# YuyaW-0118/Sparse-Matrix-Linear-Equations

Measured on AMD Instinct MI355X. Metric: fp64 SpMV GFLOP/s + achieved HBM GB/s vs roofline; CG iters/sec, higher is better.
Workload: dtype f64; 1 GPU; merge-path CSR SpMV fp64, 1 RHS, batch of 4 pwtk-shaped matrices per step per GPU (configs[1]); m=217918, nnz=11524432, batch=4, parallelism=independent SpMV batches, 1 GPU(s)

## Files before the change

sparse-matrix-linear-equations_amd/csrc/mspmv_internal.h:

```cpp
#pragma once

#include <hip/hip_runtime.h>

#include <cstdint>
#include <map>
#include <string>
#include <type_traits>
#include <utility>
#include <vector>

#include "mspmv.h"
#include "mspmv_host.h"

static inline hipError_t memset_sync(void *p, int value, size_t bytes)
{
    const hipError_t e = hipMemset(p, value, bytes);
    return e == hipSuccess ? hipStreamSynchronize(nullptr) : e;
}

namespace mspmv {

constexpr int kBlock = 256;
constexpr unsigned kFaultTicket = 1u;
constexpr int kNnzPad = 16;
// ... 214 lines not shown
    double last_tile_kernel_ms = 0.0;
    int last_kernels_per_call = 1;
    void *d_flush = nullptr;
    size_t flush_cap = 0;
    mspmv::ResidentCg *rcg = nullptr;
    std::string last_cg_kernel;
    std::string last_solver_product;
    int spmv_onewave = -1;
    int spmv_slab = -1;
    int spmv_runs = -1;
    int spmm_slab[5] = {-1, -1, -1, -1, -1};
    int dia = -1;
};

namespace mspmv {
mspmv_status host_pattern(mspmv_handle_s *h, const int **ro, const int **ci);
bool host_pattern_resident(const mspmv_handle_s *h);
struct PatternScope {
    mspmv_handle_s *h;
    bool own;
    explicit PatternScope(mspmv_handle_s *hh) : h(hh), own(!hh->pat_scope) { hh->pat_scope = true; }
    ~PatternScope()
    {
        if (own) {
            h->pat_scope = false;
            std::vector<int>().swap(h->pat_ro);
            std::vector<int>().swap(h->pat_ci);
        }
    }
};
}

namespace mspmv {

struct TriFactor {
    unsigned long long gen = mspmv_next_generation();
    int device = 0;
    int n = 0;
    int *d_lro = nullptr, *d_lci = nullptr;
    double *d_lva = nullptr;
    int *d_uro = nullptr, *d_uci = nullptr;
    double *d_uva = nullptr;
    int *d_fwd_order = nullptr;
    int *d_bwd_order = nullptr;
    double *d_y = nullptr;
    size_t y_cap = 0;
    int num_colors = 0;
    bool l_diag = false;
    std::vector<int> color_off, perm;
    std::vector<int> lmax, umax;
    int *d_perm = nullptr;
};

}

struct mspmv_ic0_s : mspmv::TriFactor {};
struct mspmv_ilu0_s : mspmv::TriFactor {
    double *d_hat = nullptr;
    size_t hat_cap = 0;
};

namespace mspmv {

hipError_t tri_apply(const TriFactor *t, const double *d_src, double *d_dst, int L, CgControl *ctrl, hipStream_t s);
hipError_t tri_solve(const TriFactor *t, int which, const double *d_b, double *d_x, int L, CgControl *ctrl,
                     hipStream_t s);
mspmv_status tri_workspace(TriFactor *t, size_t elems, const char *what);
mspmv_status ilu0_workspace(mspmv_ilu0_s *ilu, size_t elems);
void tri_graph_key(const TriFactor *t, std::vector<const void *> &key);
hipError_t launch_color_trsv(const TriFactor *t, bool upper, const double *d_b, double *d_x, int L,
                             const CgControl *ctrl, hipStream_t s);
hipError_t launch_color_apply(const TriFactor *t, const double *d_src, double *d_dst, int L, const CgControl *ctrl,
                              hipStream_t s);

constexpr int kSlabPlanKey = -1;
constexpr int kRunPlanKey = -2;
mspmv_status build_slab_plan(mspmv_handle_s *h, TilePlan &p, double min_nnz_per_block = 0.0, int cfg = 0,
                             bool groups = false, int num_groups = 0);
void free_slab(SlabData *s);
hipError_t launch_slab(mspmv_handle_s *h, const TilePlan &plan, const double *d_x, double *d_y);
std::string slab_kernel_name(const mspmv_handle_s *h);
inline int slab_mm_key(int L) { return -(1 << 20) - L; }
const SlabMmCfg &slab_mm_cfg(int L, int which = -1);
mspmv_status build_slab_mm_plan(mspmv_handle_s *h, int L, TilePlan &p);
hipError_t launch_slab_mm(mspmv_handle_s *h, const TilePlan &plan, const double *d_X, double *d_Y, int L, int ld,
                          const CgControl *ctrl);
std::string slab_mm_kernel_name(const mspmv_handle_s *h, const TilePlan &plan);
mspmv_status plan_split_rows(TilePlan &p, const std::vector<int2> &hb, const std::vector<unsigned char> &hs);

constexpr int kDiaPlanKey = -3;
mspmv_status build_dia_plan(mspmv_handle_s *h, TilePlan &p, double min_fill, double min_window_fill);
void free_dia(DiaData *d);
hipError_t launch_dia(mspmv_handle_s *h, const TilePlan &plan, const double *d_X, double *d_Y, int L, int ld,
                      const CgControl *ctrl, double *partials = nullptr, long long row_off = 0,
                      hipStream_t stream = nullptr);
std::string dia_kernel_name(const mspmv_handle_s *h, int L);
hipError_t launch_cg1_dia(mspmv_handle_s *h, const TilePlan &plan, const double *rp_old, double *rp_new, double *d_x,
                          int parity, int nblk, double tol, int *nslots);
hipError_t launch_cg1_tile(mspmv_handle_s *h, const TilePlan &plan, const double *rp_old, double *rp_new, double *d_x,
                           int parity, int nblk, double tol, int *nslots);
bool dia_spmm_enabled();
bool dia_dot_fused();

hipError_t launch_merge_coords(const int *d_row_offsets, int m, int nnz, long long diag_step, int num_parts,
                               int2 *d_out, hipStream_t s);
hipError_t launch_tile_modes(const int *d_row_offsets, const int2 *d_bounds, const unsigned char *d_split,
                             int num_tiles, int L, unsigned char *d_modes, hipStream_t s, int lanes = kBlock);
int spmv_items_per_thread();
inline int l_index(int L) { return L == 1 ? 0 : L == 2 ? 1 : L == 4 ? 2 : L == 8 ? 3 : 4; }
hipError_t launch_snap(const int *d_row_offsets, int m, int2 *d_bounds, unsigned char *d_split, int num_tiles,
                       int snap, hipStream_t s);
hipError_t launch_pack_cols16(const int *d_cols, const int2 *d_bounds, int num_tiles, int *d_colbase,
                              unsigned short *d_cols16, hipStream_t s);
bool spmv_blocks_enabled();
bool spmm_blk_enabled();
constexpr int kBlkRunRows = 6;
constexpr int kBlkPerTile = 64;
constexpr int kBlkPlanChunks = 16;
constexpr int kBlkTileChunks = 8;
hipError_t launch_build_blocks(const int *d_row_offsets, const int *d_cols, const int2 *d_bounds,
                               const unsigned char *d_split, const int *d_colbase, int num_tiles, uint4 *d_blk,
                               hipStream_t s, int max_chunks = 8);
hipError_t launch_fill_pcols(const uint4 *d_blk, int blk_stride, const int2 *d_bounds,
                             const unsigned short *d_cols16, int num_tiles, unsigned short *d_pcols, hipStream_t s);
constexpr int kRecDwords = 16;
constexpr int kRecEntries = 12;
constexpr unsigned kRecEscape = 1u << 7;

__host__ __device__ inline int blk_rec_pos(int di)
{
    return (di & ~7) | ((di & 3) << 1) | ((di >> 2) & 1);
}

__host__ __device__ inline bool blk_rec_encode(const unsigned short *P, int wc, unsigned *ent)
{
    for (int e = 0; e < kRecEntries; ++e)
        ent[e] = 0u;
    int ne = 0;
    for (int q = 0; q < wc;) {
        int len = 1;
        while (q + len < wc && (int)P[q + len] == (int)P[q] + len)
            ++len;
        if (ne == kRecEntries) {
            for (int e = 0; e < kRecEntries; ++e)
                ent[e] = 0u;
            return false;
        }
        ent[ne++] = (unsigned)P[q] | ((unsigned)len << 16) | ((unsigned)q << 24);
        q += len;
    }
    return true;
}

template <typename F>
__host__ __device__ inline unsigned blk_rec_find(F &&ent, int q, int &e)
{
    e = 0;
    unsigned E = ent(0);
#pragma unroll
    for (int step = 8; step > 0; step >>= 1) {
        const int c = e + step;
        const bool in = c < kRecEntries;
        const unsigned Ec = ent(in ? c : e);
        if (in && (int)((Ec - 1u) >> 24) <= q) {
            e = c;
            E = Ec;
        }
    }
    return E;
}

__host__ __device__ inline unsigned blk_rec_decode(const unsigned *ent, int wc, int q)
{
    q = q < wc ? q : wc - 1;
    q = q < 0 ? 0 : q;
    int e;
    const unsigned E = blk_rec_find([&](int i) { return ent[i]; }, q, e);
    return (E & 0xffffu) + (unsigned)q - (E >> 24);
}

hipError_t launch_fill_recs(const uint4 *d_blk, int blk_stride, const unsigned short *d_pcols, int num_tiles,
                            unsigned *d_recs, int *d_counts, hipStream_t s);
hipError_t launch_build_dict(const int *d_cols, const int2 *d_bounds, int num_tiles, int max_items, int *d_dict,
                             int *d_ndict, unsigned short *d_idx16, hipStream_t s, bool multi, int L = 1);
constexpr int kSpmmDictBytes = 16384;
constexpr int kSpmmDict8Bytes = 0;
constexpr int spmm_dict_bytes(int L) { return L == 16 ? kSpmmDictBytes : L == 8 ? kSpmmDict8Bytes : 0; }
constexpr int spmm_dict_max(int L) { return spmm_dict_bytes(L) / (8 * L); }
hipError_t launch_spmm(mspmv_handle_s *h, const TilePlan &plan, const double *d_X, double *d_Y, int L,
                       int *kernels_launched, int ld = 0);
hipError_t launch_panel_copy(const double *src, int lds, double *dst, int ldd, long long rows, int cols, int dcols,
                             hipStream_t s);
hipError_t launch_spmm_tile_only(mspmv_handle_s *h, const TilePlan &plan, const double *d_X, double *d_Y, int L,
                                 int ld = 0, CgControl *ctrl = nullptr);
int tile_items_for(int L);
inline int plan_key(int L) { return L == 16 ? tile_items_for(16) + 1 : tile_items_for(L); }
int spmv_tile_blocks_per_cu();
hipError_t launch_stream_read(const double *p, size_t bytes, int num_cus, hipStream_t s);
std::string spmv_kernel_name(const mspmv_handle_s *h);
std::string spmm_kernel_name(const mspmv_handle_s *h, const TilePlan &plan, int L);
std::string solver_product_kernel_name(const mspmv_handle_s *h, const TilePlan &plan, const TilePlan *splan, int L);
bool stream_nt(const mspmv_handle_s *h);

using NativeWidths = std::integer_sequence<int, 1, 2, 4, 8, 16>;
template <typename F, int... N>
inline hipError_t dispatch_width(int L, F &&f, std::integer_sequence<int, N...>)
{
    hipError_t e = hipErrorInvalidValue;
    (void)((L == N && ((e = f(std::integral_constant<int, N>{})), true)) || ...);
    return e;
}
template <typename F>
inline hipError_t dispatch_L(int L, F &&f)
{
    return dispatch_width(L, f, NativeWidths{});
}
inline bool supported_L(int L)
{
    return dispatch_L(L, [](auto) { return hipSuccess; }) == hipSuccess;
}
template <typename F>
inline auto dispatch_bool(bool flag, F &&f)
{
    return flag ? f(std::true_type{}) : f(std::false_type{});
}

hipError_t launch_cg_init(mspmv_handle_s *h, const double *d_b, double *d_x, int L, double tol, int nblk);
hipError_t launch_spmv_tile_stamped(mspmv_handle_s *h, const TilePlan &plan, const double *d_x, double *d_y,
                                   unsigned long long *d_stamps);
hipError_t launch_cg_iteration(mspmv_handle_s *h, const TilePlan &plan, const TilePlan *splan, bool dot_fused,
                               double *d_x, int L, int parity, int nblk, double tol);
int cg_update_blocks(long long elems, int num_cus);
hipError_t launch_solver_product(mspmv_handle_s *h, const TilePlan &plan, const TilePlan *splan, const double *d_X,
                                 double *d_Y, int L);
hipError_t launch_bicgstab_init(mspmv_handle_s *h, const double *d_b, double *d_x, int L, double tol, int nblk);
hipError_t launch_bicgstab_iteration(mspmv_handle_s *h, const TilePlan &plan, const TilePlan *splan, double *d_x, int L,
                                     int nblk, double tol);
hipError_t launch_pbicgstab_iteration(mspmv_handle_s *h, mspmv_ilu0_s *ilu, const TilePlan &plan,
                                      const TilePlan *splan, double *d_x, int L, int nblk, double tol);
int cg_batch_iters(long long m, long long nnz, int L);
bool cg_split_iteration(int L);
int cg1_blocks(long long m);
hipError_t launch_cg1_init(mspmv_handle_s *h, const double *d_b, double *d_x, int nblk);
hipError_t launch_cg1_finish(mspmv_handle_s *h, double *d_x, int parity, int nblk);
bool cg_resident_enabled();
bool cg_resident_pipelined();
mspmv_status resident_prepare(mspmv_handle_s *h, ResidentCg **out);
void resident_free(ResidentCg *r);
hipError_t launch_cg_resident(mspmv_handle_s *h, ResidentCg *r, const double *d_b, double *d_x, int max_iters,
                              double tol, unsigned long long *d_stamps = nullptr, int stamp_iters = 0);
hipError_t launch_cg_xflush(mspmv_handle_s *h, double *d_x, int L, int nblk);
inline void consumer_level(int nslots, int stop, int L, long long *off, int *count)
{
    long long o = 0;
    int c = nslots;
    while (c > stop) {
        o += (long long)c * L;
        c = (c + kSlotGroup - 1) / kSlotGroup;
    }
    *off = o;
    *count = c;
}

struct CgVecArgs {
    long long n_elems;
    double *x;
    double *r;
    const double *p;
    double *p0;
    const double *ap;
    CgScalars *scal;
    CgControl *ctrl;
    unsigned char *conv;
    double *partials;
    double *hist;
    int hist_cap;
    double tol;
    const double *red_in;
    double *red_out;
    unsigned *gtickets;
    int pcg;
    int lazy_x;
    int rev;
};
enum class CgVecPass {
    InitPartials,
    InitFinish,
    PUpdate,
    XrUpdate,
    Finish,
};
hipError_t launch_dist_vec(CgVecPass pass, const CgVecArgs &a, int L, int nblk, double *p, hipStream_t s);
hipError_t launch_dist_pack(const double *p, const int *idx, long long n_elems, int L, double *send,
                            const CgControl *ctrl, hipStream_t s);
hipError_t launch_spmm_dot(mspmv_handle_s *h, const TilePlan &plan, const double *d_X, double *d_Y, int L,
                           CgControl *ctrl, double *partials, unsigned *gtickets, double *dot_out,
                           CgScalars *scal = nullptr, const unsigned char *conv = nullptr, int fold_mode = -1);
hipError_t launch_spmm_dot_tiles(mspmv_handle_s *h, const TilePlan &plan, const double *d_X, double *d_Y, int L,
                                 CgControl *ctrl, double *partials, hipStream_t s, long long row_off);
hipError_t launch_fold_dot(int T, int L, double *partials, unsigned *gtickets, double *dot_out, CgScalars *scal,
                           const unsigned char *conv, CgControl *ctrl, int fold_mode, hipStream_t s);
mspmv_status solver_plan(mspmv_handle_s *h, int L, const TilePlan **out);
mspmv_status product_plan(mspmv_handle_s *h, int L, const TilePlan **out);
mspmv_status window_plan(mspmv_handle_s *h, int L, const TilePlan **out);
void free_plan(TilePlan &p);
void drop_plans(mspmv_handle_s *h);
inline int native_chunk(int left)
{
    int w = 16;
    while (w > left)
        w >>= 1;
    return w;
}
mspmv_status csr_create_on_stream(const mspmv_csr_d *host, int device, hipStream_t stream, mspmv_handle *out);
mspmv_status csr_create_view(mspmv_handle parent, int row_lo, int row_hi, const int *host_row_offsets,
                             mspmv_handle *out);
mspmv_status time_spmm_batch(int count, const mspmv_handle *hs, const double *const *d_X, double *const *d_Y, int L,
                             int reps, double *step_ms, double *tile_kernel_ms, int *kernels_per_step, bool overlap);
hipError_t launch_pcg_init(mspmv_handle_s *h, mspmv_handle_s *hm, const TilePlan &mplan, const double *d_b,
                           double *d_x, int L, double tol, int nblk);
hipError_t launch_pcg_iteration(mspmv_handle_s *h, mspmv_handle_s *hm, const TilePlan &plan, const TilePlan &mplan,
                                double *d_x, int L, int nblk, double tol);
hipError_t launch_pcg_ic0_init(mspmv_handle_s *h, mspmv_ic0_s *ic, const double *d_b, double *d_x, int L, double tol,
                               int nblk);
hipError_t launch_pcg_ic0_iteration(mspmv_handle_s *h, mspmv_ic0_s *ic, const TilePlan &plan, double *d_x, int L,
                                    int nblk, double tol);
inline size_t partials_capacity(size_t slots, int L) { return (slots + slots / (kSlotGroup - 1) + 8) * L; }
inline size_t gtickets_capacity(size_t slots) { return (slots / (kSlotGroup - 1) + 8) * kTicketStride; }

#define HIP_TRY(expr)                                                                              \
// ... 63 lines not shown
```

sparse-matrix-linear-equations_amd/csrc/mspmv_kernels.hip:

```cpp
#include "mspmv_internal.h"
#include "mspmv_device.h"

#include <algorithm>
#include <type_traits>
#include <cmath>
#include <cstdio>
#include <cstdlib>

namespace mspmv {


template <typename... KArgs, typename... Args>
static void ggl(void (*kernel)(KArgs...), dim3 grid, dim3 block, hipStream_t s, Args... args)
{
    hipLaunchKernelGGL(kernel, grid, block, 0, s, args...);
}

template <bool NT, typename T>
__device__ __forceinline__ T ld_stream(const T *p)
{
    if (NT)
        return __builtin_nontemporal_load(p);
    return *p;
}
// ... 548 lines not shown
        const int q = q0 + (int)threadIdx.x + TB * (ubase + u);
        if (q > qlast)
            continue;
        const int k0 = W * q - n0;
#pragma unroll
        for (int e = 0; e < W; ++e) {
            const double v = (e & 1) ? st.v[u][e >> 1].y : st.v[u][e >> 1].x;
            if (k0 + e >= 0 && k0 + e < nnzt)
                s_prod[pslot(k0 + e)] = v * st.x[u][e];
        }
    }
}

template <int NJ, bool CG, bool NT>
__device__ __forceinline__ void stage_products(const TileArgs &a, int n0, int nnzt, double beta, double *s_prod)
{
    StageRegs<NJ, CG> st;
    stage_issue<NJ, CG, NT>(a, n0, nnzt, -1, st);
    stage_store<NJ, CG>(st, nnzt, beta, s_prod);
}

template <int NJ, bool NT, int TB>
__device__ __forceinline__ void dict_stage(const TileArgs &a, double *s_prod, int nd, int n0, int nnzt)
{
    constexpr int DJ = 3;
    const int tid = threadIdx.x;
    int ix[NJ];
    double v[NJ];
    int dc[DJ];
    double dx[DJ];
#pragma unroll
    for (int u = 0; u < DJ; ++u)
        dc[u] = ld_stream<NT>(a.dict + n0 + min(tid + u * TB, nd - 1));
#pragma unroll
    for (int j = 0; j < NJ; ++j)
        ix[j] = ld_stream<NT>(a.idx16 + n0 + min(tid + j * TB, nnzt - 1));
#pragma unroll
    for (int j = 0; j < NJ; ++j)
        v[j] = ld_stream<NT>(a.vals + n0 + min(tid + j * TB, nnzt - 1));
#pragma unroll
    for (int u = 0; u < DJ; ++u)
        dx[u] = a.x[dc[u]];
    double *s_x = s_prod;
#pragma unroll
    for (int u = 0; u < DJ; ++u)
        if (tid + u * TB < nd)
            s_x[tid + u * TB] = dx[u];
    for (int d = tid + DJ * TB; d < nd; d += TB)
        s_x[d] = a.x[a.dict[n0 + d]];
    tile_sync<TB>();
    double pr[NJ];
#pragma unroll
    for (int j = 0; j < NJ; ++j)
        pr[j] = v[j] * s_x[ix[j]];
    tile_sync<TB>();
#pragma unroll
    for (int j = 0; j < NJ; ++j) {
        const int k = tid + j * TB;
        if (k < nnzt)
            s_prod[pslot(k)] = pr[j];
    }
}

template <bool CG>
struct BlkRegs {
    int c[2];
    double v[2][kBlkRows];
    double xv[2];
    double pv[CG ? 2 : 1];
};

__device__ __forceinline__ uint4 blk_read(const uint4 &bd, int di)
{
    return make_uint4((unsigned)__builtin_amdgcn_readlane((int)bd.x, di),
                      (unsigned)__builtin_amdgcn_readlane((int)bd.y, di),
                      (unsigned)__builtin_amdgcn_readlane((int)bd.z, di),
                      (unsigned)__builtin_amdgcn_readlane((int)bd.w, di));
}

__device__ __forceinline__ const unsigned short *blk_slot(const TileArgs &a, int t, int di)
{
    return a.pcols + ((size_t)t * a.blk_stride + di) * 64;
}

template <bool CG, bool NT, int TB, typename Head>
__device__ __forceinline__ void blk_stage(const TileArgs &a, int t, const uint4 &bd, int nd, int n0, int colbase,
                                          double *s_prod, double &beta, Head &&head)
{
    constexpr int NW = TB / 64;
    const int lane = threadIdx.x & 63;
    const int wave = __builtin_amdgcn_readfirstlane((int)(threadIdx.x >> 6));
    for (int round = 0; round * 2 * NW < nd; ++round) {
        BlkRegs<CG> st;
#pragma unroll
        for (int s = 0; s < 2; ++s) {
            const int di = wave + NW * (2 * round + s);
            st.c[s] = 0;
#pragma unroll
            for (int i = 0; i < kBlkRows; ++i)
                st.v[s][i] = 0.0;
            if (di < nd) {
                const uint4 d = blk_read(bd, di);
                const int vofs = d.x & 0xffff, j0 = (d.x >> 16) & 255, wc = d.x >> 24;
                const int h = d.y & 15;
                const int j = j0 + lane;
                int start = 0;
#pragma unroll
                for (int i = 0; i < kBlkRows; ++i) {
                    const int len = blk_len(d, i);
                    if (i < h && j < len)
                        st.v[s][i] = ld_stream<NT>(a.vals + n0 + vofs + start + j);
                    start += i < h ? len : 0;
                }
                if (lane < wc)
                    st.c[s] = colbase + (int)ld_stream<NT>(blk_slot(a, t, di) + lane);
            }
        }
#pragma unroll
        for (int s = 0; s < 2; ++s) {
            if constexpr (CG) {
                const double2 v = cg_rp(a, st.c[s]);
                st.xv[s] = v.x;
                st.pv[s] = v.y;
            } else {
                st.xv[s] = a.x[st.c[s]];
            }
        }
        if (round == 0 && !head())
            return;
#pragma unroll
        for (int s = 0; s < 2; ++s) {
            const int di = wave + NW * (2 * round + s);
            if (di < nd) {
                const uint4 d = blk_read(bd, di);
                const int vofs = d.x & 0xffff, j0 = (d.x >> 16) & 255;
                const int h = d.y & 15;
                const int j = j0 + lane;
                double x = st.xv[s];
                if (CG)
                    x = x + beta * st.pv[s];
                int start = 0;
#pragma unroll
                for (int i = 0; i < kBlkRows; ++i) {
                    const int len = blk_len(d, i);
                    if (i < h && j < len)
                        s_prod[pslot(vofs + start + j)] = st.v[s][i] * x;
                    start += i < h ? len : 0;
                }
            }
        }
    }
}

__device__ __forceinline__ double rows8_sum(const double (&p)[kBlkRows])
{
    const int lane = threadIdx.x & 63;
    const bool b5 = lane & 32, b4 = lane & 16, b3 = lane & 8;
    double q4[4], q2[2];
#pragma unroll
    for (int k = 0; k < 4; ++k)
        q4[k] = (b5 ? p[k + 4] : p[k]) + __shfl_xor(b5 ? p[k] : p[k + 4], 32);
#pragma unroll
    for (int k = 0; k < 2; ++k)
        q2[k] = (b4 ? q4[k + 2] : q4[k]) + __shfl_xor(b4 ? q4[k] : q4[k + 2], 16);
    double v = (b3 ? q2[1] : q2[0]) + __shfl_xor(b3 ? q2[0] : q2[1], 8);
    v += __shfl_xor(v, 4);
    v += __shfl_xor(v, 2);
    v += __shfl_xor(v, 1);
    return v;
}

__device__ __forceinline__ double rows8_sum32(const double (&p)[kBlkRows])
{
    const int lane = threadIdx.x & 63;
    const bool b4 = lane & 16, b3 = lane & 8, b2 = lane & 4;
    double q4[4], q2[2];
#pragma unroll
    for (int k = 0; k < 4; ++k)
        q4[k] = (b4 ? p[k + 4] : p[k]) + __shfl_xor(b4 ? p[k] : p[k + 4], 16);
#pragma unroll
    for (int k = 0; k < 2; ++k)
        q2[k] = (b3 ? q4[k + 2] : q4[k]) + __shfl_xor(b3 ? q4[k] : q4[k + 2], 8);
    double v = (b2 ? q2[1] : q2[0]) + __shfl_xor(b2 ? q2[0] : q2[1], 4);
    v += __shfl_xor(v, 2);
    v += __shfl_xor(v, 1);
    return v;
}

template <bool NT>
__device__ __forceinline__ unsigned blk_pair_rec(const TileArgs &a, int t, int round)
{
    const int lane = threadIdx.x & 63;
    const int slot = 8 * round + 2 * (int)(threadIdx.x >> 6) + (lane >> 5);
    return ld_stream<NT>(a.recs + ((size_t)t * a.blk_stride + slot) * kRecDwords + (lane & 15));
}

template <bool NT, int KR>
__device__ __forceinline__ void blk_rows_pair(const TileArgs &a, int t, unsigned rec, int nd, int r0, int n0,
                                              int colbase)
{
    constexpr int NW = kBlock / 64;
    const int lane = threadIdx.x & 63;
    const int half = lane >> 5, hl = lane & 31;
    const int wave = __builtin_amdgcn_readfirstlane((int)(threadIdx.x >> 6));
    for (int round = 0; round * 2 * NW < nd; ++round) {
        if (round > 0)
            rec = blk_pair_rec<NT>(a, t, round);
        const int di = wave + NW * (2 * round + half);
        const bool valid = di < nd;
        auto dword = [&](int k) { return (unsigned)__shfl((int)rec, (lane & 32) + k); };
        const uint4 d = make_uint4(dword(0), dword(1), dword(2), dword(3));
        const int vofs = d.x & 0xffff, wc = d.x >> 24;
        const int h = d.y & 15, rofs = d.y >> 16;
        double2 v[KR];
        bool in0[KR], in1[KR];
        int start = 0;
#pragma unroll
        for (int i = 0; i < KR; ++i) {
            const int len = blk_len(d, i);
            in0[i] = valid && i < h && 2 * hl < len;
            in1[i] = valid && i < h && 2 * hl + 1 < len;
            v[i] = make_double2(0.0, 0.0);
            if (in0[i])
                v[i] = ld_stream<NT>(reinterpret_cast<const double2 *>(a.vals + n0 + vofs + start + 2 * hl));
            start += i < h ? len : 0;
        }
        const int q = max(min(2 * hl, wc - 1), 0);
        int e;
        const unsigned E = blk_rec_find([&](int i) { return dword(4 + i); }, q, e);
        const unsigned En = dword(4 + min(e + 1, kRecEntries - 1));
        int c0 = colbase + (int)((E & 0xffffu) + (unsigned)q - (E >> 24));
        int c1 = c0 + 1;
        if (2 * hl + 1 < wc && 2 * hl + 1 == (int)((E >> 24) + ((E >> 16) & 255u)))
            c1 = colbase + (int)(En & 0xffffu);
        if (d.y & kRecEscape) {
            const int p = (d.y >> 4) & 7;
            int pstart = 0;
#pragma unroll
            for (int i = 0; i < KR - 1; ++i)
                pstart += i < p ? blk_len(d, i) : 0;
            unsigned cc = 0u;
            if (2 * hl < wc)
                cc = ld_stream<NT>(reinterpret_cast<const unsigned *>(a.cols16 + n0 + vofs + pstart + 2 * hl));
            c0 = colbase + (int)(cc & 0xffffu);
            c1 = 2 * hl + 1 < wc ? colbase + (int)(cc >> 16) : c0 + 1;
        }
        const int base = min(c0, a.n - 2);
        const double2 xx = *reinterpret_cast<const double2 *>(a.x + base);
        const double x0 = base == c0 ? xx.x : xx.y;
        double x1 = xx.y;
        if (c1 != c0 + 1)
            x1 = a.x[c1];
        double pr[kBlkRows];
#pragma unroll
        for (int i = 0; i < kBlkRows; ++i)
            pr[i] = i < KR ? (in0[i] ? v[i].x * x0 : 0.0) + (in1[i] ? v[i].y * x1 : 0.0) : 0.0;
        const double sum = rows8_sum32(pr);
        const int myrow = hl >> 2;
        if (valid && (hl & 3) == 0 && myrow < h)
            a.y[r0 + rofs + myrow] = sum;
    }
}

template <int MODE, bool NT, int TB, typename Head>
__device__ __forceinline__ void blk_rows(const TileArgs &a, int t, const uint4 &bd, int nd, int r0, int n0,
                                         int colbase, double &beta, double &dot, Head &&head)
{
    constexpr bool CG = MODE == kModeCg;
    constexpr int NW = TB / 64;
    const int lane = threadIdx.x & 63;
    const int wave = __builtin_amdgcn_readfirstlane((int)(threadIdx.x >> 6));
    const int myrow = lane >> 3;
    for (int round = 0; round * 2 * NW < nd; ++round) {
        BlkRegs<CG> st;
        double2 ro[2];
#pragma unroll
        for (int s = 0; s < 2; ++s) {
            const int di = wave + NW * (2 * round + s);
            st.c[s] = 0;
            ro[s] = make_double2(0.0, 0.0);
#pragma unroll
            for (int i = 0; i < kBlkRows; ++i)
                st.v[s][i] = 0.0;
            if (di < nd) {
                const uint4 d = blk_read(bd, di);
                const int vofs = d.x & 0xffff, wc = d.x >> 24;
                const int h = d.y & 15, rofs = d.y >> 16;
                int start = 0;
#pragma unroll
                for (int i = 0; i < kBlkRows; ++i) {
                    const int len = blk_len(d, i);
                    if (i < h && lane < len)
                        st.v[s][i] = ld_stream<NT>(a.vals + n0 + vofs + start + lane);
                    start += i < h ? len : 0;
                }
                if (lane < wc)
                    st.c[s] = colbase + (int)ld_stream<NT>(blk_slot(a, t, di) + lane);
                if (MODE != kModeSpmv && (lane & 7) == 0 && myrow < h) {
                    const int R = r0 + rofs + myrow;
                    if constexpr (CG)
                        ro[s] = cg_rp(a, R);
                    else
                        ro[s].x = a.xr[R];
                }
            }
        }
#pragma unroll
        for (int s = 0; s < 2; ++s) {
            if constexpr (CG) {
                const double2 v = cg_rp(a, st.c[s]);
                st.xv[s] = v.x;
                st.pv[s] = v.y;
            } else {
                st.xv[s] = a.x[st.c[s]];
            }
        }
        if (round == 0 && !head())
            return;
#pragma unroll
        for (int s = 0; s < 2; ++s) {
            const int di = wave + NW * (2 * round + s);
            if (di < nd) {
                const uint4 d = blk_read(bd, di);
                const int h = d.y & 15, rofs = d.y >> 16;
                double x = st.xv[s];
                if (CG)
                    x = x + beta * st.pv[s];
                double pr[kBlkRows];
#pragma unroll
                for (int i = 0; i < kBlkRows; ++i)
                    pr[i] = (i < h && lane < blk_len(d, i)) ? st.v[s][i] * x : 0.0;
                const double sum = rows8_sum(pr);
                if ((lane & 7) == 0 && myrow < h) {
                    const int R = r0 + rofs + myrow;
                    a.y[R] = sum;
                    if constexpr (CG) {
                        const double pn = ro[s].x + beta * ro[s].y;
                        cg_pstore(a, R, pn);
                        dot += pn * sum;
                    } else if constexpr (MODE == kModeDot) {
                        dot += ro[s].x * sum;
                    }
                }
            }
        }
    }
}

template <int IPT, int TB = kBlock>
struct SpmvSmem {
    static constexpr int TILE = TB * IPT;
    static constexpr int MAXI = TILE + TILE / kSnapDiv;
    static constexpr int MAXJ = (MAXI + TB - 1) / TB;
    double prod[MAXI + 8];
    double red[TB / 64];
    int last;
    __device__ __forceinline__ int *rowend(int nnzt) { return reinterpret_cast<int *>(prod + ((nnzt + 7) & ~7)); }
    __device__ __forceinline__ double *scratch_val() { return prod; }
    __device__ __forceinline__ int *scratch_row() { return reinterpret_cast<int *>(prod + TB); }
    static_assert(MAXI + 8 >= TB + TB / 2, "scratch must fit the product buffer");
};

template <int IPT, int MODE, int TB = kBlock, bool FIX = true>
__device__ __forceinline__ void walk_tile(const TileArgs &a, SpmvSmem<IPT, TB> &sm, int t, int r0, int n0, int nrows,
                                          int nnzt, bool tail, double beta, double &dot)
{
    constexpr int MAXJ = SpmvSmem<IPT, TB>::MAXJ;
    const int tid = threadIdx.x;
    const int *rend = sm.rowend(nnzt);
    const int items = nrows + nnzt;
    const int ipt = (items + TB - 1) / TB;
    const int d0 = min(tid * ipt, items);
    int cx, cy, ex = nrows, ey = nnzt;
    lds_search(d0, rend, nrows, nnzt, cx, cy);
    if (tid + 1 < TB)
        lds_search(min(d0 + ipt, items), rend, nrows, nnzt, ex, ey);
    const bool need_cin = (cx < ex) && (cy > (cx == 0 ? 0 : rend[cx - 1]));
    double pr[MAXJ];
    if (ey > cy) {
#pragma unroll
        for (int j = 0; j < MAXJ; ++j)
            pr[j] = sm.prod[pslot(min(cy + j, ey - 1))];
    }
// ... 684 lines not shown
        s_rowend[tid] = re0 - n0;
    for (int i = kBlock + tid; i < nrows; i += kBlock)
        s_rowend[i] = a.row_offsets[r0 + 1 + i] - n0;
    __syncthreads();
    if (stopped)
        return;

    double2 dot = make_double2(0.0, 0.0);
    if (rmode != 0) {
        if (DICT && nd > 0)
            spmm_group_rows<L, true, FIX>(a, s_col, s_val, s_rowend, t, r0, nrows, nnzt, rmode - 1, s_panel);
        else
            spmm_group_rows<L, false, FIX>(a, s_col, s_val, s_rowend, t, r0, nrows, nnzt, rmode - 1);
    } else {
    const int ipt = (items + NG - 1) / NG;
    const int d0 = min(g * ipt, items);
    const int d1 = min(d0 + ipt, items);
    int cx, cy, ex, ey;
    lds_search(d0, s_rowend, nrows, nnzt, cx, cy);
    lds_search(d1, s_rowend, nrows, nnzt, ex, ey);
    const bool need_cin = (cx < ex) && (cy > (cx == 0 ? 0 : s_rowend[cx - 1]));

    auto write_row = [&](int row, double2 val) {
        __builtin_nontemporal_store(v2d_t{val.x, val.y},
                                    reinterpret_cast<v2d_t *>(FIX && row == 0 ? a.y0 + 2 * lane
                                                                              : a.y + (size_t)(r0 + row) * a.ld + 2 * lane));
    };

    double2 run = make_double2(0.0, 0.0);
    bool first = true, pend = false;
    int prow = 0;
    double2 pval = make_double2(0.0, 0.0);
    constexpr int WJ = 4;
#pragma unroll
    for (int j0 = 0; j0 < MAXJ; j0 += WJ) {
        if (cy + j0 >= ey)
            break;
        double2 xr[WJ];
        double vv[WJ];
#pragma unroll
        for (int jj = 0; jj < WJ; ++jj) {
            const int k = min(cy + j0 + jj, ey - 1);
            vv[jj] = s_val[k];
            xr[jj] = *reinterpret_cast<const double2 *>(a.x + (size_t)s_col[k] * a.ld + 2 * lane);
        }
#pragma unroll
        for (int jj = 0; jj < WJ; ++jj) {
            const int k = cy + j0 + jj;
            if (j0 + jj < MAXJ && k < ey) {
                while (cx < ex && s_rowend[cx] <= k) {
                    if (first && need_cin) {
                        pend = true;
                        prow = cx;
                        pval = run;
                    } else {
                        write_row(cx, run);
                    }
                    first = false;
                    run = make_double2(0.0, 0.0);
                    ++cx;
                }
                run.x += vv[jj] * xr[jj].x;
                run.y += vv[jj] * xr[jj].y;
            }
        }
    }
    while (cx < ex) {
        if (first && need_cin) {
            pend = true;
            prow = cx;
            pval = run;
        } else {
            write_row(cx, run);
        }
        first = false;
        run = make_double2(0.0, 0.0);
        ++cx;
    }
    if (lane == 0)
        s_crow[g] = ex;
    s_cval[g * GL + lane] = run;
    __syncthreads();

    if (pend) {
        int j0 = g - 1;
        while (j0 > 0 && s_crow[j0 - 1] == prow)
            --j0;
        double2 acc = s_cval[j0 * GL + lane];
        for (int u = j0 + 1; u < g; ++u) {
            const double2 c = s_cval[u * GL + lane];
            acc.x += c.x;
            acc.y += c.y;
        }
        acc.x += pval.x;
        acc.y += pval.y;
        write_row(prow, acc);
    }
    if (g == NG - 1 && a.split[t + 1]) {
        int j0 = NG - 1;
        while (j0 > 0 && s_crow[j0 - 1] == nrows)
            --j0;
        double2 acc = s_cval[j0 * GL + lane];
        for (int u = j0 + 1; u < NG; ++u) {
            const double2 c = s_cval[u * GL + lane];
            acc.x += c.x;
            acc.y += c.y;
        }
        store_sc1_2(a.carry_val + (size_t)t * L + 2 * lane, acc);
    }
    }

    if (MODE == kModeDot) {
        asm volatile("s_waitcnt vmcnt(0)" ::: "memory");
        __syncthreads();
        const int npair = (nrows + (a.split[t + 1] ? 1 : 0)) * GL;
        for (int e = tid; e < npair; e += kBlock) {
            const int row = e / GL;
            const size_t off = (size_t)(r0 + row) * a.ld + 2 * lane;
            const double2 ap = *reinterpret_cast<const double2 *>(
                row < nrows ? (FIX && row == 0 ? a.y0 + 2 * lane : a.y + off) : a.carry_val + (size_t)t * L + 2 * lane);
            const double2 xx = *reinterpret_cast<const double2 *>(a.xr + off);
            dot.x += xx.x * ap.x;
            dot.y += xx.y * ap.y;
        }
    }
    if (MODE != kModeSpmv) {
#pragma unroll
        for (int off = 32; off >= GL; off >>= 1) {
            dot.x += __shfl_xor(dot.x, off);
            dot.y += __shfl_xor(dot.y, off);
        }
        if ((tid & 63) < GL)
            s_red2[tid >> 6][lane] = dot;
        __syncthreads();
        if (tid < GL) {
            double2 tsum = s_red2[0][tid];
#pragma unroll
            for (int w = 1; w < kBlock / 64; ++w) {
                tsum.x += s_red2[w][tid].x;
                tsum.y += s_red2[w][tid].y;
            }
            a.partials[(size_t)t * L + 2 * tid] = tsum.x;
            a.partials[(size_t)t * L + 2 * tid + 1] = tsum.y;
        }
    }
    if constexpr (FIX)
        close_split_rows<kBlock>(a, t, s_fix, L, a.ld);
}

template <int GL>
__device__ __forceinline__ double2 rows8_sum2(const double2 (&p)[kBlkRows])
{
    const int lane = threadIdx.x & 63;
    const bool b5 = lane & 32, b4 = lane & 16, b3 = lane & 8;
    auto sx = [](double2 v, int off) { return make_double2(__shfl_xor(v.x, off), __shfl_xor(v.y, off)); };
    auto add = [](double2 u, double2 v) { return make_double2(u.x + v.x, u.y + v.y); };
    double2 q4[4], q2[2];
#pragma unroll
    for (int k = 0; k < 4; ++k)
        q4[k] = add(b5 ? p[k + 4] : p[k], sx(b5 ? p[k] : p[k + 4], 32));
#pragma unroll
    for (int k = 0; k < 2; ++k)
        q2[k] = add(b4 ? q4[k + 2] : q4[k], sx(b4 ? q4[k] : q4[k + 2], 16));
    double2 v = add(b3 ? q2[1] : q2[0], sx(b3 ? q2[0] : q2[1], 8));
#pragma unroll
    for (int off = 4; off >= GL; off >>= 1)
        v = add(v, sx(v, off));
    return v;
}

constexpr int spmm_blk_waves(int L, int MODE, int KR) { return MODE == 0 && KR <= 6 && L >= 4 ? 8 : 1; }
template <int L, int MODE, bool NT, int KR = kBlkRows>
__global__ __launch_bounds__(kBlock) __attribute__((amdgpu_waves_per_eu(spmm_blk_waves(L, MODE, KR)))) void
k_spmm_blk(TileArgs a)
{
    static_assert(MODE != kModeCg, "multi-RHS CG runs the split iteration (MODE 2)");
    constexpr int GL = L / 2;
    constexpr int NGW = 64 / GL;
    constexpr int PB = L >= 16 ? 2 : 1;
    __shared__ double2 s_red2[MODE == kModeDot ? kBlock / 64 : 1][GL];
    __shared__ __attribute__((aligned(16))) double s_v[kBlock / 64][kBlkRows][64];
    __shared__ int s_c[kBlock / 64][64];
    const int stopped = (MODE != kModeSpmv || a.ctrl) ? a.ctrl->done : 0;
    const int tid = threadIdx.x, lane = tid & 63;
    const int g = lane / GL, c = lane % GL;
    const int t = xcd_tile(blockIdx.x, a.num_tiles);
    const int2 b0 = a.bounds[t];
    const int r0 = b0.x, n0 = b0.y;
    const int colbase = a.colbase[t];
    const uint4 bd = lane < a.blk_stride ? a.blk[(size_t)t * a.blk_stride + lane] : make_uint4(0u, 0u, 0u, 0u);
    const int nd = (int)(((unsigned)__builtin_amdgcn_readfirstlane((int)bd.y) >> 8) & 255u);
    const int wave = __builtin_amdgcn_readfirstlane((int)(tid >> 6));
    double2 dot = make_double2(0.0, 0.0);
    auto fetch = [&](int di, int &cj, double (&vr)[KR]) {
        const uint4 d = blk_read(bd, di);
        const int vofs = d.x & 0xffff, wc = d.x >> 24;
        const int h = d.y & 15;
        int start[KR];
        int acc_s = 0;
#pragma unroll
        for (int i = 0; i < KR; ++i) {
            start[i] = acc_s;
            acc_s += i < h ? blk_len(d, i) : 0;
        }
        cj = lane < wc ? colbase + (int)ld_stream<NT>(blk_slot(a, t, di) + lane) : 0;
#pragma unroll
        for (int i = 0; i < KR; ++i)
            vr[i] = (i < h && lane < blk_len(d, i)) ? ld_stream<NT>(a.vals + n0 + vofs + start[i] + lane) : 0.0;
    };
    for (int di = wave; di < nd && !stopped; di += kBlock / 64) {
        const uint4 d = blk_read(bd, di);
        const int wc = d.x >> 24;
        const int h = d.y & 15, rofs = d.y >> 16;
        {
            int colj;
            double vrow[KR];
            fetch(di, colj, vrow);
            s_c[wave][lane] = colj;
#pragma unroll
            for (int i = 0; i < KR; ++i)
                s_v[wave][i][lane] = vrow[i];
            __builtin_amdgcn_wave_barrier();
        }
        const int ri = lane >> 3;
        const bool store = (lane & 7) < GL && ri < h;
        double2 xx = make_double2(0.0, 0.0);
        if (MODE == kModeDot && store)
            xx = *reinterpret_cast<const double2 *>(a.xr + (size_t)(r0 + rofs + ri) * a.ld + 2 * c);
        double2 acc[kBlkRows];
#pragma unroll
        for (int i = 0; i < kBlkRows; ++i)
            acc[i] = make_double2(0.0, 0.0);
        int minlen = 64;
#pragma unroll
        for (int i = 0; i < KR; ++i)
            minlen = i < h ? min(minlen, blk_len(d, i)) : minlen;
        int pb = 0;
        for (; (pb + PB) * NGW <= minlen; pb += PB) {
            int cq[PB];
#pragma unroll
            for (int q = 0; q < PB; ++q)
                cq[q] = s_c[wave][((pb + q) * NGW + g) & 63];
            double2 xv[PB];
#pragma unroll
            for (int q = 0; q < PB; ++q)
                xv[q] = *reinterpret_cast<const double2 *>(a.x + (size_t)cq[q] * a.ld + 2 * c);
#pragma unroll
            for (int q = 0; q < PB; ++q) {
                const int j = (pb + q) * NGW + g;
#pragma unroll
                for (int i = 0; i < KR; ++i) {
                    const double v = s_v[wave][i][j & 63];
                    acc[i].x = __builtin_fma(v, xv[q].x, acc[i].x);
                    acc[i].y = __builtin_fma(v, xv[q].y, acc[i].y);
                }
                asm volatile("" ::: "memory");
            }
        }
        for (; pb * NGW < wc; ++pb) {
            const int j = pb * NGW + g;
            const int cq = s_c[wave][j & 63];
            const double2 xv = *reinterpret_cast<const double2 *>(a.x + (size_t)cq * a.ld + 2 * c);
#pragma unroll
            for (int i = 0; i < KR; ++i) {
                const double v = s_v[wave][i][j & 63];
                const bool on = i < h && j < blk_len(d, i);
                acc[i].x += on ? v * xv.x : 0.0;
                acc[i].y += on ? v * xv.y : 0.0;
            }
        }
        const double2 row = rows8_sum2<GL>(acc);
        if (store) {
            *reinterpret_cast<double2 *>(a.y + (size_t)(r0 + rofs + ri) * a.ld + 2 * c) = row;
            if (MODE == kModeDot) {
                dot.x += xx.x * row.x;
                dot.y += xx.y * row.y;
            }
        }
    }
    if constexpr (MODE == kModeDot) {
        if (stopped)
            return;
#pragma unroll
        for (int off = 32; off >= GL; off >>= 1) {
            dot.x += __shfl_xor(dot.x, off);
            dot.y += __shfl_xor(dot.y, off);
        }
        if (lane < GL)
            s_red2[tid >> 6][lane] = dot;
        __syncthreads();
        if (tid < GL) {
            double2 tsum = s_red2[0][tid];
#pragma unroll
            for (int w = 1; w < kBlock / 64; ++w) {
                tsum.x += s_red2[w][tid].x;
                tsum.y += s_red2[w][tid].y;
            }
            a.partials[(size_t)t * L + 2 * tid] = tsum.x;
            a.partials[(size_t)t * L + 2 * tid + 1] = tsum.y;
        }
    }
}

__global__ void k_flush(double *p, long long n, double v)
{
    for (long long i = (long long)blockIdx.x * blockDim.x + threadIdx.x; i < n; i += (long long)gridDim.x * blockDim.x)
        p[i] = v;
}
__global__ __launch_bounds__(kBlock) void k_stream_read(const double2 *p, long long n2, double *sink)
{
    constexpr int U = 8;
    const long long per = (n2 + gridDim.x - 1) / gridDim.x;
    const long long b = (long long)blockIdx.x * per;
    const long long e = b + per < n2 ? b + per : n2;
    const long long step = (long long)kBlock * U;
    auto ld = [&](long long i) { return i < e ? ld_stream<true>(p + i) : make_double2(0.0, 0.0); };
    double acc = 0.0;
    double2 t0[U], t1[U];
    long long i = b + threadIdx.x;
#pragma unroll
// ... 495 lines not shown
```

Measured before the change: 1338 GFLOP/s.

## Replace shuffle-based reductions and record decode with DPP/permlane cross-lane ops

Replaces __shfl_xor-based (ds_bpermute) butterfly reductions in rows8_sum, rows8_sum32 and rows8_sum2 with permlane32/16_swap and DPP row operations. It also broadcasts record dwords with DPP row_bcast instead of shuffles. The binary search over run-length column records becomes a DPP-OR'd bitmask of run starts plus a popcount. The goal is to cut LDS-crossbar shuffle latency and instruction count in the per-block inner loop, at the cost of relying on gfx950-specific intrinsics and subtle lane-mask correctness.

```diff
diff --git a/sparse-matrix-linear-equations_amd/csrc/mspmv_internal.h b/sparse-matrix-linear-equations_amd/csrc/mspmv_internal.h
--- a/sparse-matrix-linear-equations_amd/csrc/mspmv_internal.h
+++ b/sparse-matrix-linear-equations_amd/csrc/mspmv_internal.h
@@ -390,30 +390,25 @@
     return true;
 }
 
-template <typename F>
-__host__ __device__ inline unsigned blk_rec_find(F &&ent, int q, int &e)
-{
-    e = 0;
-    unsigned E = ent(0);
-#pragma unroll
-    for (int step = 8; step > 0; step >>= 1) {
-        const int c = e + step;
-        const bool in = c < kRecEntries;
-        const unsigned Ec = ent(in ? c : e);
-        if (in && (int)((Ec - 1u) >> 24) <= q) {
-            e = c;
-            E = Ec;
-        }
-    }
-    return E;
+__host__ __device__ inline unsigned long long blk_rec_start_bit(unsigned E)
+{
+    return (E >> 16) & 255u ? 1ull << ((E >> 24) & 63u) : 0ull;
+}
+__host__ __device__ inline int blk_rec_index(unsigned long long starts, int q)
+{
+    const unsigned long long low = (2ull << q) - 1ull;
+    const int n = __builtin_popcountll(starts & low);
+    return n > 0 ? n - 1 : 0;
 }
 
 __host__ __device__ inline unsigned blk_rec_decode(const unsigned *ent, int wc, int q)
 {
     q = q < wc ? q : wc - 1;
     q = q < 0 ? 0 : q;
-    int e;
-    const unsigned E = blk_rec_find([&](int i) { return ent[i]; }, q, e);
+    unsigned long long starts = 0ull;
+    for (int i = 0; i < kRecEntries; ++i)
+        starts |= blk_rec_start_bit(ent[i]);
+    const unsigned E = ent[blk_rec_index(starts, q)];
     return (E & 0xffffu) + (unsigned)q - (E >> 24);
 }
 
diff --git a/sparse-matrix-linear-equations_amd/csrc/mspmv_kernels.hip b/sparse-matrix-linear-equations_amd/csrc/mspmv_kernels.hip
--- a/sparse-matrix-linear-equations_amd/csrc/mspmv_kernels.hip
+++ b/sparse-matrix-linear-equations_amd/csrc/mspmv_kernels.hip
@@ -724,38 +724,106 @@
     }
 }
 
+
+template <int CTRL, int BANKS>
+__device__ __forceinline__ int dpp_new(int src)
+{
+    return __builtin_amdgcn_mov_dpp(src, CTRL, 0xf, BANKS, false);
+}
+template <int CTRL, int BANKS = 0xf>
+__device__ __forceinline__ int dpp_into(int old, int src)
+{
+    return __builtin_amdgcn_update_dpp(old, src, CTRL, 0xf, BANKS, false);
+}
+
+template <int K>
+__device__ __forceinline__ unsigned row_bcast(unsigned v)
+{
+    return (unsigned)dpp_into<0x150 + K>(0, (int)v);
+}
+
+template <int GROUP>
+__device__ __forceinline__ void swap_halves(double &a, double &b)
+{
+    const unsigned al = (unsigned)__double2loint(a), ah = (unsigned)__double2hiint(a);
+    const unsigned bl = (unsigned)__double2loint(b), bh = (unsigned)__double2hiint(b);
+    if constexpr (GROUP == 32) {
+        const auto lo = __builtin_amdgcn_permlane32_swap(al, bl, false, false);
+        const auto hi = __builtin_amdgcn_permlane32_swap(ah, bh, false, false);
+        a = __hiloint2double((int)hi[0], (int)lo[0]);
+        b = __hiloint2double((int)hi[1], (int)lo[1]);
+    } else {
+        static_assert(GROUP == 16, "swap_halves: 32- or 16-lane groups");
+        const auto lo = __builtin_amdgcn_permlane16_swap(al, bl, false, false);
+        const auto hi = __builtin_amdgcn_permlane16_swap(ah, bh, false, false);
+        a = __hiloint2double((int)hi[0], (int)lo[0]);
+        b = __hiloint2double((int)hi[1], (int)lo[1]);
+    }
+}
+
+__device__ __forceinline__ double recv_xor8(double a, double b)
+{
+    int lo = dpp_new<0x128, 0x3>(__double2loint(a)), hi = dpp_new<0x128, 0x3>(__double2hiint(a));
+    lo = dpp_into<0x128, 0xc>(lo, __double2loint(b));
+    hi = dpp_into<0x128, 0xc>(hi, __double2hiint(b));
+    return __hiloint2double(hi, lo);
+}
+__device__ __forceinline__ double recv_xor4(double a, double b)
+{
+    int lo = dpp_new<0x104, 0x5>(__double2loint(a)), hi = dpp_new<0x104, 0x5>(__double2hiint(a));
+    lo = dpp_into<0x114, 0xa>(lo, __double2loint(b));
+    hi = dpp_into<0x114, 0xa>(hi, __double2hiint(b));
+    return __hiloint2double(hi, lo);
+}
+template <int OFF>
+__device__ __forceinline__ double recv_quad(double v)
+{
+    static_assert(OFF == 2 || OFF == 1, "recv_quad: inside a quad");
+    constexpr int ctrl = OFF == 2 ? 0x4e : 0xb1;
+    return __hiloint2double(dpp_new<ctrl, 0xf>(__double2hiint(v)), dpp_new<ctrl, 0xf>(__double2loint(v)));
+}
+
 __device__ __forceinline__ double rows8_sum(const double (&p)[kBlkRows])
 {
     const int lane = threadIdx.x & 63;
-    const bool b5 = lane & 32, b4 = lane & 16, b3 = lane & 8;
+    const bool b3 = lane & 8;
     double q4[4], q2[2];
 #pragma unroll
-    for (int k = 0; k < 4; ++k)
-        q4[k] = (b5 ? p[k + 4] : p[k]) + __shfl_xor(b5 ? p[k] : p[k + 4], 32);
+    for (int k = 0; k < 4; ++k) {
+        double a = p[k], b = p[k + 4];
+        swap_halves<32>(a, b);
+        q4[k] = a + b;
+    }
+#pragma unroll
+    for (int k = 0; k < 2; ++k) {
+        double a = q4[k], b = q4[k + 2];
+        swap_halves<16>(a, b);
+        q2[k] = a + b;
+    }
+    double v = (b3 ? q2[1] : q2[0]) + recv_xor8(q2[0], q2[1]);
+    v += recv_xor4(v, v);
+    v += recv_quad<2>(v);
+    v += recv_quad<1>(v);
+    return v;
+}
+
+__device__ __forceinline__ double rows8_sum32(const double (&p)[kBlkRows])
+{
+    const int lane = threadIdx.x & 63;
+    const bool b3 = lane & 8, b2 = lane & 4;
+    double q4[4], q2[2];
+#pragma unroll
+    for (int k = 0; k < 4; ++k) {
+        double a = p[k], b = p[k + 4];
+        swap_halves<16>(a, b);
+        q4[k] = a + b;
+    }
 #pragma unroll
     for (int k = 0; k < 2; ++k)
-        q2[k] = (b4 ? q4[k + 2] : q4[k]) + __shfl_xor(b4 ? q4[k] : q4[k + 2], 16);
-    double v = (b3 ? q2[1] : q2[0]) + __shfl_xor(b3 ? q2[0] : q2[1], 8);
-    v += __shfl_xor(v, 4);
-    v += __shfl_xor(v, 2);
-    v += __shfl_xor(v, 1);
-    return v;
-}
-
-__device__ __forceinline__ double rows8_sum32(const double (&p)[kBlkRows])
-{
-    const int lane = threadIdx.x & 63;
-    const bool b4 = lane & 16, b3 = lane & 8, b2 = lane & 4;
-    double q4[4], q2[2];
-#pragma unroll
-    for (int k = 0; k < 4; ++k)
-        q4[k] = (b4 ? p[k + 4] : p[k]) + __shfl_xor(b4 ? p[k] : p[k + 4], 16);
-#pragma unroll
-    for (int k = 0; k < 2; ++k)
-        q2[k] = (b3 ? q4[k + 2] : q4[k]) + __shfl_xor(b3 ? q4[k] : q4[k + 2], 8);
-    double v = (b2 ? q2[1] : q2[0]) + __shfl_xor(b2 ? q2[0] : q2[1], 4);
-    v += __shfl_xor(v, 2);
-    v += __shfl_xor(v, 1);
+        q2[k] = (b3 ? q4[k + 2] : q4[k]) + recv_xor8(q4[k], q4[k + 2]);
+    double v = (b2 ? q2[1] : q2[0]) + recv_xor4(q2[0], q2[1]);
+    v += recv_quad<2>(v);
+    v += recv_quad<1>(v);
     return v;
 }
 
@@ -780,8 +848,7 @@
             rec = blk_pair_rec<NT>(a, t, round);
         const int di = wave + NW * (2 * round + half);
         const bool valid = di < nd;
-        auto dword = [&](int k) { return (unsigned)__shfl((int)rec, (lane & 32) + k); };
-        const uint4 d = make_uint4(dword(0), dword(1), dword(2), dword(3));
+        const uint4 d = make_uint4(row_bcast<0>(rec), row_bcast<1>(rec), row_bcast<2>(rec), row_bcast<3>(rec));
         const int vofs = d.x & 0xffff, wc = d.x >> 24;
         const int h = d.y & 15, rofs = d.y >> 16;
         double2 v[KR];
@@ -798,9 +865,21 @@
             start += i < h ? len : 0;
         }
         const int q = max(min(2 * hl, wc - 1), 0);
-        int e;
-        const unsigned E = blk_rec_find([&](int i) { return dword(4 + i); }, q, e);
-        const unsigned En = dword(4 + min(e + 1, kRecEntries - 1));
+        const unsigned long long bit = (lane & 15) >= 4 ? blk_rec_start_bit(rec) : 0ull;
+        unsigned mlo = (unsigned)bit, mhi = (unsigned)(bit >> 32);
+        mlo |= (unsigned)dpp_into<0x128>(0, (int)mlo);
+        mhi |= (unsigned)dpp_into<0x128>(0, (int)mhi);
+        mlo |= (unsigned)dpp_into<0x124>(0, (int)mlo);
+        mhi |= (unsigned)dpp_into<0x124>(0, (int)mhi);
+        mlo |= (unsigned)dpp_into<0x122>(0, (int)mlo);
+        mhi |= (unsigned)dpp_into<0x122>(0, (int)mhi);
+        mlo |= (unsigned)dpp_into<0x121>(0, (int)mlo);
+        mhi |= (unsigned)dpp_into<0x121>(0, (int)mhi);
+        const int e = blk_rec_index((unsigned long long)mhi << 32 | mlo, q);
+        const int ent0 = ((lane & ~15) + 4) << 2;
+        const unsigned E = (unsigned)__builtin_amdgcn_ds_bpermute(ent0 + (e << 2), (int)rec);
+        const unsigned En =
+            (unsigned)__builtin_amdgcn_ds_bpermute(ent0 + (min(e + 1, kRecEntries - 1) << 2), (int)rec);
         int c0 = colbase + (int)((E & 0xffffu) + (unsigned)q - (E >> 24));
         int c1 = c0 + 1;
         if (2 * hl + 1 < wc && 2 * hl + 1 == (int)((E >> 24) + ((E >> 16) & 255u)))
@@ -1791,20 +1870,30 @@
 __device__ __forceinline__ double2 rows8_sum2(const double2 (&p)[kBlkRows])
 {
     const int lane = threadIdx.x & 63;
-    const bool b5 = lane & 32, b4 = lane & 16, b3 = lane & 8;
-    auto sx = [](double2 v, int off) { return make_double2(__shfl_xor(v.x, off), __shfl_xor(v.y, off)); };
+    const bool b3 = lane & 8;
     auto add = [](double2 u, double2 v) { return make_double2(u.x + v.x, u.y + v.y); };
     double2 q4[4], q2[2];
 #pragma unroll
-    for (int k = 0; k < 4; ++k)
-        q4[k] = add(b5 ? p[k + 4] : p[k], sx(b5 ? p[k] : p[k + 4], 32));
-#pragma unroll
-    for (int k = 0; k < 2; ++k)
-        q2[k] = add(b4 ? q4[k + 2] : q4[k], sx(b4 ? q4[k] : q4[k + 2], 16));
-    double2 v = add(b3 ? q2[1] : q2[0], sx(b3 ? q2[0] : q2[1], 8));
-#pragma unroll
-    for (int off = 4; off >= GL; off >>= 1)
-        v = add(v, sx(v, off));
+    for (int k = 0; k < 4; ++k) {
+        double2 u = p[k], w = p[k + 4];
+        swap_halves<32>(u.x, w.x);
+        swap_halves<32>(u.y, w.y);
+        q4[k] = add(u, w);
+    }
+#pragma unroll
+    for (int k = 0; k < 2; ++k) {
+        double2 u = q4[k], w = q4[k + 2];
+        swap_halves<16>(u.x, w.x);
+        swap_halves<16>(u.y, w.y);
+        q2[k] = add(u, w);
+    }
+    double2 v = add(b3 ? q2[1] : q2[0], make_double2(recv_xor8(q2[0].x, q2[1].x), recv_xor8(q2[0].y, q2[1].y)));
+    if constexpr (GL <= 4)
+        v = add(v, make_double2(recv_xor4(v.x, v.x), recv_xor4(v.y, v.y)));
+    if constexpr (GL <= 2)
+        v = add(v, make_double2(recv_quad<2>(v.x), recv_quad<2>(v.y)));
+    if constexpr (GL <= 1)
+        v = add(v, make_double2(recv_quad<1>(v.x), recv_quad<1>(v.y)));
     return v;
 }
 
```

Result: no change. 1330 GFLOP/s (-0.6%).
